# APRIL-ZJU/Ctrl-VIO

Measured on AMD Instinct MI355X. Metric: sliding-window solves/sec (10 KF, 200 lm, 2000 IMU), higher is better.
Workload: dtype f64; 1 GPU; config2: 10 KF / 200 landmarks / 2000 IMU sliding window (K = 24 knots, 814 reprojection blocks), <= 15 LM iterations (Ceres 1.14 trust region + projected line search); distinct_windows_per_gpu=64, streams_per_gpu=4, concurrent_solves_per_gpu=2

## Files before the change

ctrl-vio_amd/csrc/factors.hpp:

```cpp
#pragma once
#include "so3.hpp"

namespace ctv {

struct Knots4 {
  Q4 q[4];
  V3 p[4];
};

struct SegConst {
  V3 d[3];
  M3 JrI[3];
  CTV_DI M3 jri(int i) const { return JrI[i]; }
};
struct SegConstLazy {
  V3 d[3];
  const double *tab;
  CTV_DI M3 jri(int i) const {
    M3 J;
#pragma unroll
    for (int e = 0; e < 9; ++e) J.m[e] = tab[9 * i + e];
    return J;
  }
};
struct SegConstS {
  V3 d[3];
  M3 JrI[3];
  CTV_DI const M3 &jri(int i) const { return JrI[i]; }
};
CTV_DI void seg_const_lazy(const double *kd, const double *kjri, SegConstLazy &sc) {
#pragma unroll
  for (int i = 0; i < 3; ++i) sc.d[i] = mk(kd[3 * i], kd[3 * i + 1], kd[3 * i + 2]);
  sc.tab = kjri;
}
CTV_DI void seg_const(const Knots4 &k, SegConst &sc, bool want_jac) {
#pragma unroll
  for (int i = 0; i < 3; ++i) {
    sc.d[i] = so3_log(qmul(qconj(k.q[i]), k.q[i + 1]));
    if (want_jac) sc.JrI[i] = so3_Jr_inv(sc.d[i]);
  }
}

CTV_DI void knot_pair_const(const double *qa, const double *qb, double *d3, double *jri9) {
  const V3 dd = so3_log(qmul(qconj(qmk(qa[0], qa[1], qa[2], qa[3])), qmk(qb[0], qb[1], qb[2], qb[3])));
  d3[0] = dd.x; d3[1] = dd.y; d3[2] = dd.z;
  if (jri9) {
    const M3 J = so3_Jr_inv(mk(dd.x, dd.y, dd.z));
#pragma unroll
    for (int e = 0; e < 9; ++e) jri9[e] = J.m[e];
  }
}
CTV_DI void seg_const_load(const double *kd, const double *kjri, SegConst &sc, bool want_jac) {
#pragma unroll
  for (int i = 0; i < 3; ++i) {
    sc.d[i] = mk(kd[3 * i], kd[3 * i + 1], kd[3 * i + 2]);
    if (want_jac) {
#pragma unroll
      for (int e = 0; e < 9; ++e) sc.JrI[i].m[e] = kjri[9 * i + e];
    }
  }
}

struct ImuJac {
  M3 Jw[4], Ja[4];
  M3 Rinv_g;
  double lamA[4];
};

template <class SC> 
CTV_DI void imu_eval_core(const Knots4 &k, const SC &sc, double u, double idt, V3 gravity, const double bias[6],
                          const double gyro[3], const double acc[3], const double w[6], const M3 &RrefT, double r[6], bool want_jac, ImuJac &J) {
  double lamR[4], lamW[4];
  double (&lamA)[4] = J.lamA;
  basis<false, 2>(u, idt * idt, lamA);
  basis<true, 0>(u, 1.0, lamR);
  basis<true, 1>(u, idt, lamW);

  V3 accel = mk(0, 0, 0);
#pragma unroll
  for (int i = 0; i < 4; ++i) accel = accel + lamA[i] * k.p[i];

  Q4 Ainv[3], accq = qmk(0, 0, 0, 1);
  M3 Apost[4], JrK[3];
  Apost[3] = m3_id();
#pragma unroll
  for (int i = 2; i >= 0; --i) {
    const V3 nkd = (-lamR[i + 1]) * sc.d[i];
    Ainv[i] = so3_exp(nkd);
    accq = qmul_unit(accq, Ainv[i]);
    if (want_jac) { Apost[i] = q2R(accq); JrK[i] = so3_Jr(nkd); }
  }
  V3 om[4];
  om[0] = mk(0, 0, 0);
#pragma unroll
  for (int i = 0; i < 3; ++i) om[i + 1] = qrot(Ainv[i], om[i]) + lamW[i + 1] * sc.d[i];

  const Q4 Rinv_q = qmul_unit(accq, qconj(k.q[0]));
  const V3 ag = accel + gravity;
  const V3 a_pred = qrot(Rinv_q, ag);
  r[0] = w[0] * (om[3].x - (gyro[0] - bias[0]));
  r[1] = w[1] * (om[3].y - (gyro[1] - bias[1]));
  r[2] = w[2] * (om[3].z - (gyro[2] - bias[2]));
  r[3] = w[3] * (a_pred.x - (acc[0] - bias[3]));
  r[4] = w[4] * (a_pred.y - (acc[1] - bias[4]));
  r[5] = w[5] * (a_pred.z - (acc[2] - bias[5]));
  if (!want_jac) return;

  M3 (&Jw)[4] = J.Jw;
  M3 (&Ja)[4] = J.Ja;
#pragma unroll
  for (int i = 0; i < 4; ++i) { Jw[i] = m3_zero(); Ja[i] = m3_zero(); }
  {
    M3 dod = scale(Apost[1], lamW[1]);
#pragma unroll
    for (int i = 0; i < 3; ++i) {
      if (i > 0) dod = add(scale(mul(mul_hat(Apost[i], om[i]), JrK[i]), lamR[i + 1]), scale(Apost[i + 1], lamW[i + 1]));
      const M3 JrIi = sc.jri(i);
      Jw[i] = sub(Jw[i], mulT(dod, JrIi));
      Jw[i + 1] = add(Jw[i + 1], mul(dod, JrIi));
    }
  }
  const M3 Rinv = q2R(Rinv_q);
  J.Rinv_g = mul(Rinv, RrefT);
  {
    const M3 lhs = mul_hat(Rinv, ag);
    M3 Racc = q2R(k.q[0]);
    Ja[0] = add(Ja[0], mul(lhs, Racc));
#pragma unroll
    for (int i = 0; i < 3; ++i) {
      if (i > 0) Racc = mulT(Racc, q2R(Ainv[i - 1]));
      const M3 dad = scale(mul(mul(lhs, Racc), JrK[i]), lamR[i + 1]);
      const M3 JrIi = sc.jri(i);
      Ja[i] = sub(Ja[i], mulT(dad, JrIi));
      Ja[i + 1] = add(Ja[i + 1], mul(dad, JrIi));
    }
  }
}

CTV_DI void imu_row_gyro2(const M3 (&Jw)[4], const double w[6], const double r[6], int a, double out[16]) {
#pragma unroll
  for (int kk = 0; kk < 4; ++kk)
#pragma unroll
    for (int b = 0; b < 3; ++b) out[3 * kk + b] = w[a] * Jw[kk].m[3 * a + b];
  out[12] = out[13] = out[14] = 0.0;
  out[12 + a] = w[a];
  out[15] = r[a];
}

struct ImuMid3 {
  M3 Apost[3];
  M3 JrK[3];
  V3 om1, om2;
  V3 b[3];
  double lamR[4], lamW[4], lamA[4];
};
template <class SC> 
CTV_DI void imu_eval_values3(const double *gc, const SC &sc, double u, double idt, const double gyro[3], const double acc[3], const double w[6], double r[6], ImuMid3 &md) {
  basis<false, 2>(u, idt * idt, md.lamA);
  basis<true, 0>(u, 1.0, md.lamR);
  basis<true, 1>(u, idt, md.lamW);
  V3 ag = mk(gc[21], gc[22], gc[23]);
#pragma unroll
  for (int i = 1; i < 4; ++i) ag = ag + md.lamA[i] * mk(gc[3 * i], gc[3 * i + 1], gc[3 * i + 2]);
  Q4 Ainv[3], accq;
#pragma unroll
  for (int i = 2; i >= 0; --i) {
    const V3 nkd = (-md.lamR[i + 1]) * sc.d[i];
    Ainv[i] = so3_exp_small(nkd);
    accq = i == 2 ? Ainv[2] : qmul_unit(accq, Ainv[i]);
    md.Apost[i] = q2R(accq);
    md.JrK[i] = so3_Jr_small(nkd);
  }
  V3 om3;
  md.om1 = md.lamW[1] * sc.d[0];
  md.om2 = qrot(Ainv[1], md.om1) + md.lamW[2] * sc.d[1];
  om3 = qrot(Ainv[2], md.om2) + md.lamW[3] * sc.d[2];
  md.b[0] = mk(gc[12] * ag.x + gc[13] * ag.y + gc[14] * ag.z, gc[15] * ag.x + gc[16] * ag.y + gc[17] * ag.z,
                  gc[18] * ag.x + gc[19] * ag.y + gc[20] * ag.z);
  md.b[1] = qrot(Ainv[0], md.b[0]);
  md.b[2] = qrot(Ainv[1], md.b[1]);
  const V3 a_pred = qrot(Ainv[2], md.b[2]);
  r[0] = w[0] * (om3.x - (gyro[0] - gc[24]));
  r[1] = w[1] * (om3.y - (gyro[1] - gc[25]));
  r[2] = w[2] * (om3.z - (gyro[2] - gc[26]));
  r[3] = w[3] * (a_pred.x - (acc[0] - gc[27]));
  r[4] = w[4] * (a_pred.y - (acc[1] - gc[28]));
  r[5] = w[5] * (a_pred.z - (acc[2] - gc[29]));
}
template <class SC> CTV_DI void imu_apply_pair(const M3 &M, const SC &sc, int i, M3 &Ji, M3 &Ji1, bool first) {
  const M3 JrIi = sc.jri(i);
  const M3 A = mulT(M, JrIi), B = mul(M, JrIi);
#pragma unroll
  for (int e = 0; e < 9; ++e) { Ji.m[e] = first ? -A.m[e] : Ji.m[e] - A.m[e]; Ji1.m[e] = B.m[e]; }
}
template <class SC> CTV_DI void imu_jac_gyro3(const ImuMid3 &md, const SC &sc, M3 (&Jw)[4]) {
  imu_apply_pair(scale(md.Apost[1], md.lamW[1]), sc, 0, Jw[0], Jw[1], true);
  imu_apply_pair(add(scale(mul(mul_hat(md.Apost[1], md.om1), md.JrK[1]), md.lamR[2]), scale(md.Apost[2], md.lamW[2])), sc, 1, Jw[1], Jw[2], false);
  M3 dod = scale(mul(mul_hat(md.Apost[2], md.om2), md.JrK[2]), md.lamR[3]);
  dod.m[0] += md.lamW[3]; dod.m[4] += md.lamW[3]; dod.m[8] += md.lamW[3];
  imu_apply_pair(dod, sc, 2, Jw[2], Jw[3], false);
}
template <class SC> 
CTV_DI void imu_jac_accel3(const ImuMid3 &md, const SC &sc, const double *gc, M3 (&Ja)[4], M3 &Rinv_g) {
#pragma unroll
  for (int i = 0; i < 3; ++i)
#pragma unroll
    for (int j = 0; j < 3; ++j)
      Rinv_g.m[3 * i + j] = md.Apost[0].m[3 * i] * gc[12 + j] + md.Apost[0].m[3 * i + 1] * gc[15 + j] + md.Apost[0].m[3 * i + 2] * gc[18 + j];
  Ja[0] = mul_hat(md.Apost[0], md.b[0]);
#pragma unroll
  for (int i = 0; i < 3; ++i)
    imu_apply_pair(scale(mul(mul_hat(md.Apost[i], md.b[i]), md.JrK[i]), md.lamR[i + 1]), sc, i, Ja[i], Ja[i + 1], false);
}

CTV_DI void imu_row_accel3(const M3 (&Ja)[4], const double lamA[4], const M3 &Rinv_g, const double w[6], const double r[6], int a, double out[28]) {
#pragma unroll
  for (int kk = 0; kk < 4; ++kk)
#pragma unroll
    for (int b = 0; b < 3; ++b) {
      out[3 * kk + b] = w[3 + a] * Ja[kk].m[3 * a + b];
      out[16 + 3 * kk + b] = w[3 + a] * lamA[kk] * Rinv_g.m[3 * a + b];
    }
  out[12] = out[13] = out[14] = 0.0;
  out[12 + a] = w[3 + a];
  out[15] = r[3 + a];
}
template <class Sink> CTV_DI void imu_emit_cols(const ImuJac &J, const double w[6], Sink &sink) {
#pragma unroll
  for (int kk = 0; kk < 4; ++kk)
#pragma unroll
    for (int b = 0; b < 3; ++b) {
      double c6[6], p6[6];
#pragma unroll
      for (int a = 0; a < 3; ++a) {
        c6[a] = w[a] * J.Jw[kk].m[3 * a + b];
        c6[3 + a] = w[3 + a] * J.Ja[kk].m[3 * a + b];
        p6[a] = 0.0;
        p6[3 + a] = w[3 + a] * J.lamA[kk] * J.Rinv_g.m[3 * a + b];
      }
      sink.put_col(3 * kk + b, c6);
      sink.put_col(12 + 3 * kk + b, p6);
    }
#pragma unroll
  for (int a = 0; a < 3; ++a) {
    double g6[6] = {0.0, 0.0, 0.0, 0.0, 0.0, 0.0}, h6[6] = {0.0, 0.0, 0.0, 0.0, 0.0, 0.0};
    g6[a] = w[a];
    h6[3 + a] = w[3 + a];
    sink.put_col(24 + a, g6);
    sink.put_col(27 + a, h6);
  }
}
CTV_DI void imu_row_accel(const ImuJac &J, const double w[6], const double r[6], int a, double out[32]) {
#pragma unroll
  for (int kk = 0; kk < 4; ++kk)
#pragma unroll
    for (int b = 0; b < 3; ++b) {
      out[3 * kk + b] = w[3 + a] * J.Ja[kk].m[3 * a + b];
      out[12 + 3 * kk + b] = w[3 + a] * J.lamA[kk] * J.Rinv_g.m[3 * a + b];
    }
#pragma unroll
  for (int c = 24; c < 32; ++c) out[c] = 0.0;
  out[27 + a] = w[3 + a];
  out[30] = r[3 + a];
}
CTV_DI void imu_row_gyro(const ImuJac &J, const double w[6], const double r[6], int a, double out[16]) {
#pragma unroll
  for (int kk = 0; kk < 4; ++kk)
#pragma unroll
    for (int b = 0; b < 3; ++b) out[3 * kk + b] = w[a] * J.Jw[kk].m[3 * a + b];
  out[12] = out[13] = out[14] = 0.0;
  out[12 + a] = w[a];
  out[15] = r[a];
}

template <class Sink, class SC> 
CTV_DI void imu_eval(const Knots4 &k, const SC &sc, double u, double idt, V3 gravity, const double bias[6],
                     const double gyro[3], const double acc[3], const double w[6], const M3 &RrefT, double r[6], bool want_jac, Sink &sink) {
  ImuJac J;
  imu_eval_core<SC>(k, sc, u, idt, gravity, bias, gyro, acc, w, RrefT, r, want_jac, J);
  if (want_jac) imu_emit_cols(J, w, sink);
}

template <class SC, bool SMALL = false> CTV_DI Q4 eval_Rp(const Q4 q[4], const SC &sc, double u, M3 J[4], bool want_jac) {
  double c[4];
  basis<true, 0>(u, 1.0, c);
  Q4 accq = qmk(0, 0, 0, 1);
  M3 Apost[4], JrK[3];
  Apost[3] = m3_id();
#pragma unroll
  for (int i = 2; i >= 0; --i) {
    const V3 kd = c[i + 1] * sc.d[i];
    accq = qmul_unit(accq, so3_exp_sel<SMALL>(neg(kd)));
    if (want_jac) { JrK[i] = so3_Jr_sel<SMALL>(kd); Apost[i] = q2R(accq); }
  }
  const Q4 res = qmul_unit(q[0], qconj(accq));
  if (want_jac) {
    J[0] = Apost[0];
#pragma unroll
    for (int i = 0; i < 3; ++i) {
      const M3 Jh = scale(mul(Apost[i + 1], JrK[i]), c[i + 1]);
      J[i] = sub(J[i], mulT(Jh, sc.jri(i)));
      J[i + 1] = mul(Jh, sc.jri(i));
    }
  }
  return res;
}
template <class SC, bool SMALL = false> CTV_DI Q4 eval_RTp(const Q4 q[4], const SC &sc, double u, M3 J[4], bool want_jac) {
  double c[4];
  basis<true, 0>(u, 1.0, c);
  Q4 S[4];
  M3 JrK[3];
  S[0] = q[0];
#pragma unroll
  for (int i = 0; i < 3; ++i) {
    const V3 kd = c[i + 1] * sc.d[i];
    S[i + 1] = qmul_unit(S[i], so3_exp_sel<SMALL>(kd));
    if (want_jac) JrK[i] = so3_Jr_sel<SMALL>(neg(kd));
  }
  if (want_jac) {
    J[0] = q2R(S[0]);
#pragma unroll
    for (int i = 0; i < 3; ++i) {
      const M3 Jh = scale(mul(q2R(S[i]), JrK[i]), c[i + 1]);
      J[i] = sub(J[i], mulT(Jh, sc.jri(i)));
      J[i + 1] = mul(Jh, sc.jri(i));
    }
  }
  return qconj(S[3]);
}
template <class SC, bool SMALL = false> CTV_DI V3 eval_omega(const SC &sc, double u, double idt) {
  double c[4], dc[4];
  basis<true, 0>(u, 1.0, c);
  basis<true, 1>(u, idt, dc);
  V3 rv = dc[1] * sc.d[0];
#pragma unroll
  for (int i = 1; i < 3; ++i) rv = qrot(so3_exp_sel<SMALL>((-c[i + 1]) * sc.d[i]), rv) + dc[i + 1] * sc.d[i];
  return rv;
}
template <class SC> CTV_DI Q4 eval_R(const Q4 q[4], const SC &sc, double u) {
  double c[4];
  basis<true, 0>(u, 1.0, c);
  Q4 res = q[0];
#pragma unroll
  for (int i = 0; i < 3; ++i) res = qmul_unit(res, so3_exp(c[i + 1] * sc.d[i]));
  return res;
}

template <class SC> CTV_DI void pose_jac_T(const Q4 q[4], const SC &sc, double u, bool ext_on, Q4 q_SI, V3 p_SI, double *jt) {
  M3 J[4];
  const Q4 R = eval_Rp<SC>(q, sc, u, J, true);
  double c[4];
  basis<false, 0>(u, 1.0, c);
  M3 RSI = m3_id(), X = m3_zero();
  if (ext_on) { RSI = q2R(q_SI); X = scale(mul_hat(q2R(R), p_SI), -1.0); }
#pragma unroll
  for (int k = 0; k < 4; ++k) {
    const M3 B = mul(X, J[k]);
#pragma unroll
    for (int cc = 0; cc < 3; ++cc)
#pragma unroll
      for (int a = 0; a < 3; ++a) {
        jt[(6 * k + cc) * 6 + a] = ext_on ? RSI.m[a] * J[k].m[cc] + RSI.m[3 + a] * J[k].m[3 + cc] + RSI.m[6 + a] * J[k].m[6 + cc] : J[k].m[3 * a + cc];
        jt[(6 * k + cc) * 6 + 3 + a] = ext_on ? B.m[3 * a + cc] : 0.0;
        jt[(6 * k + 3 + cc) * 6 + a] = 0.0;
        jt[(6 * k + 3 + cc) * 6 + 3 + a] = a == cc ? c[k] : 0.0;
      }
  }
}

template <class SC> CTV_DI void nav_jac_T(const Q4 q[4], const SC &sc, double u, double idt, double *jt, double cv[4]) {
  pose_jac_T(q, sc, u, false, qmk(0.0, 0.0, 0.0, 1.0), mk(0.0, 0.0, 0.0), jt);
  basis<false, 1>(u, idt, cv);
}

CTV_DI void rel_pose_jac_T(Q4 q_a, V3 p_a, Q4 q_b, V3 p_b, double *jt_a, double *jt_b, Q4 &q_ab, V3 &p_ab) {
  q_ab = qmul(qconj(q_a), q_b);
  const M3 Ra = q2R(q_a), Rab = q2R(q_ab);
  const V3 d = p_b - p_a;
  p_ab = mk(Ra.m[0] * d.x + Ra.m[3] * d.y + Ra.m[6] * d.z, Ra.m[1] * d.x + Ra.m[4] * d.y + Ra.m[7] * d.z, Ra.m[2] * d.x + Ra.m[5] * d.y + Ra.m[8] * d.z);
  if (!jt_a) return;
  for (int r = 0; r < 24; ++r) {
    double *ja = jt_a + 6 * r, *jb = jt_b + 6 * r;
    const V3 th = mk(ja[0], ja[1], ja[2]), dp = mk(ja[3], ja[4], ja[5]), db = mk(jb[3], jb[4], jb[5]);
    const V3 x = cross(p_ab, th);
#pragma unroll
    for (int a = 0; a < 3; ++a) {
      ja[a] = -(Rab.m[a] * th.x + Rab.m[3 + a] * th.y + Rab.m[6 + a] * th.z);
      ja[3 + a] = (a == 0 ? x.x : a == 1 ? x.y : x.z) - (Ra.m[a] * dp.x + Ra.m[3 + a] * dp.y + Ra.m[6 + a] * dp.z);
      jb[3 + a] = Ra.m[a] * db.x + Ra.m[3 + a] * db.y + Ra.m[6 + a] * db.z;
    }
  }
}

template <class SC, bool SMALL = false, class F> CTV_DI void eval_Rp_jac_stream(const SC &sc, double u, F &&f) {
  double c[4];
  basis<true, 0>(u, 1.0, c);
  Q4 accq = qmk(0, 0, 0, 1);
  M3 Ap = m3_id(), pending = m3_zero();
#pragma unroll
  for (int i = 2; i >= 0; --i) {
    const V3 kd = c[i + 1] * sc.d[i];
    const M3 Jh = scale(mul(Ap, so3_Jr_sel<SMALL>(kd)), c[i + 1]);
    const M3 JrIi = sc.jri(i);
    const M3 Jn = mul(Jh, JrIi);
    f(i + 1, i == 2 ? Jn : add(Jn, pending));
    pending = scale(mulT(Jh, JrIi), -1.0);
    accq = qmul_unit(accq, so3_exp_sel<SMALL>(neg(kd)));
    Ap = q2R(accq);
  }
  f(0, add(Ap, pending));
}
template <class SC, bool SMALL = false, class F> CTV_DI void eval_RTp_jac_stream(const Q4 q[4], const SC &sc, double u, F &&f) {
  double c[4];
  basis<true, 0>(u, 1.0, c);
  Q4 S = q[0];
  M3 pending = q2R(S);
#pragma unroll
  for (int i = 0; i < 3; ++i) {
    const V3 kd = c[i + 1] * sc.d[i];
    const M3 Jh = scale(mul(q2R(S), so3_Jr_sel<SMALL>(neg(kd))), c[i + 1]);
    const M3 JrIi = sc.jri(i);
    f(i, sub(pending, mulT(Jh, JrIi)));
    pending = mul(Jh, JrIi);
    S = qmul_unit(S, so3_exp_sel<SMALL>(kd));
  }
  f(3, pending);
}

constexpr int AREC = 50;
constexpr int AR_PG = 0;
constexpr int AR_GR = 3;
constexpr int AR_CP0 = 39;
constexpr int AR_Y = 43;
constexpr int AR_H = 46;

template <bool SMALL, class SC>
CTV_DI void vis_anchor_eval(const Q4 &q0, const V3 p[4], const SC &sc, double u, double idt, const Q4 &q_CI,
                            const V3 &p_CI, double pix, double piy, double rowi, double d_inv, bool want_jac, double *rec) {
  const double inv_d = 1.0 / d_inv;
  const V3 c_i = qrot(q_CI, mk(pix * inv_d, piy * inv_d, inv_d));
  const V3 p_Ii = c_i + p_CI;
  Q4 qk[4];
  qk[0] = q0;
  const Q4 S_IitoG = eval_Rp<SC, SMALL>(qk, sc, u, (M3 *)nullptr, false);
  const M3 RIiG = q2R(S_IitoG);
  double cp0[4];
  basis<false, 0>(u, 1.0, cp0);
  V3 pI = mk(0, 0, 0);
#pragma unroll
  for (int i = 0; i < 4; ++i) pI = pI + cp0[i] * p[i];
  const V3 pG = mul(RIiG, p_Ii) + pI;
  rec[AR_PG] = pG.x; rec[AR_PG + 1] = pG.y; rec[AR_PG + 2] = pG.z;
  if (!want_jac) return;
  double dcp0[4];
  basis<false, 1>(u, idt, dcp0);
  V3 v_i = mk(0, 0, 0);
#pragma unroll
  for (int i = 0; i < 4; ++i) v_i = v_i + dcp0[i] * p[i];
#pragma unroll
  for (int i = 0; i < 4; ++i) rec[AR_CP0 + i] = cp0[i];
  const V3 y = (-inv_d) * mul(RIiG, c_i);
  rec[AR_Y] = y.x; rec[AR_Y + 1] = y.y; rec[AR_Y + 2] = y.z;
  const V3 Om_i = eval_omega<SC, SMALL>(sc, u, idt);
  const V3 h = rowi * (v_i + mul(RIiG, cross(Om_i, p_Ii)));
  rec[AR_H] = h.x; rec[AR_H + 1] = h.y; rec[AR_H + 2] = h.z;
  const M3 M0 = scale(mul_hat(RIiG, p_Ii), -1.0);
  eval_Rp_jac_stream<SC, SMALL>(sc, u, [&](int kk, const M3 &Jk) {
    const M3 G = mul(M0, Jk);
#pragma unroll
    for (int b = 0; b < 3; ++b)
#pragma unroll
      for (int mm = 0; mm < 3; ++mm) rec[AR_GR + 3 * (3 * kk + b) + mm] = G.m[3 * mm + b];
  });
}

constexpr int VB_JROT = 0;
constexpr int VB_RHO = 24;
constexpr int VB_LD = 26;
constexpr int VB_RES = 28;
constexpr int VB_AT = 30;
constexpr int VB_CP1 = 36;

template <bool SMALL, class SC, class Emit>
CTV_DI double vis_block_eval(const double *rec, const Q4 &q0, const V3 p[4], const SC &sc, double u, double idt,
                             const M3 &RCIT, const V3 &p_CI, double sw, double cauchy_a, double pjx, double pjy, double rowj,
                             double r[2], bool want_jac, Emit &emit) {
  double c[4], cp1[4];
  basis<true, 0>(u, 1.0, c);
  basis<false, 0>(u, 1.0, cp1);
  Q4 A[3], S[4];
  S[0] = q0;
#pragma unroll
  for (int i = 0; i < 3; ++i) {
    A[i] = so3_exp_sel<SMALL>(c[i + 1] * sc.d[i]);
    S[i + 1] = qmul_unit(S[i], A[i]);
  }
  const Q4 S_GtoIj = qconj(S[3]);
  V3 pIj = mk(0, 0, 0);
#pragma unroll
  for (int i = 0; i < 4; ++i) pIj = pIj + cp1[i] * p[i];
  const V3 dpg = mk(rec[AR_PG], rec[AR_PG + 1], rec[AR_PG + 2]) - pIj;
  const V3 bj = qrot(S_GtoIj, dpg);
  const V3 x_j = mul(RCIT, bj - p_CI);
  const double dji = 1.0 / x_j.z;
  const double r0 = sw * (x_j.x * dji - pjx), r1 = sw * (x_j.y * dji - pjy);
  const double s = r0 * r0 + r1 * r1;
  double cost, sq = 1.0, rs = 1.0, alpha_sq = 0.0;
  if (cauchy_a > 0.0) {
    const double b = cauchy_a * cauchy_a, cc = 1.0 / b;
    const double inv = 1.0 / (1.0 + s * cc);
    cost = 0.5 * b * log1p(s * cc);
    const double rho1 = inv, rho2 = -cc * inv * inv;
    sq = sqrt(rho1);
    if (s == 0.0 || rho2 <= 0.0) { rs = sq; alpha_sq = 0.0; }
    else { const double D = 1.0 + 2.0 * s * rho2 / rho1; const double al = 1.0 - sqrt(D); rs = sq / (1.0 - al); alpha_sq = al / s; }
  } else {
    cost = 0.5 * s;
  }
  r[0] = rs * r0;
  r[1] = rs * r1;
  if (!want_jac) return cost;
  double Bt[6], At[6];
  {
    const double fx = -dji * dji * x_j.x, fy = -dji * dji * x_j.y;
#pragma unroll
    for (int k = 0; k < 3; ++k) {
      const double j0 = sw * (dji * RCIT.m[k] + fx * RCIT.m[6 + k]), j1 = sw * (dji * RCIT.m[3 + k] + fy * RCIT.m[6 + k]);
      const double rj = r0 * j0 + r1 * j1;
      Bt[k] = sq * (j0 - alpha_sq * r0 * rj);
      Bt[3 + k] = sq * (j1 - alpha_sq * r1 * rj);
    }
  }
  const M3 RGIj = q2R(S_GtoIj);
#pragma unroll
  for (int a = 0; a < 2; ++a)
#pragma unroll
    for (int k = 0; k < 3; ++k) At[3 * a + k] = Bt[3 * a] * RGIj.m[k] + Bt[3 * a + 1] * RGIj.m[3 + k] + Bt[3 * a + 2] * RGIj.m[6 + k];
  emit.put(VB_RHO, At[0] * rec[AR_Y] + At[1] * rec[AR_Y + 1] + At[2] * rec[AR_Y + 2]);
  emit.put(VB_RHO + 1, At[3] * rec[AR_Y] + At[4] * rec[AR_Y + 1] + At[5] * rec[AR_Y + 2]);
#pragma unroll
  for (int mm = 0; mm < 3; ++mm) { emit.put(VB_AT + 2 * mm, At[mm]); emit.put(VB_AT + 2 * mm + 1, At[3 + mm]); }
#pragma unroll
  for (int i = 0; i < 4; ++i) emit.put(VB_CP1 + i, cp1[i]);
  {
    double dc[4], dcp1[4];
    basis<true, 1>(u, idt, dc);
    basis<false, 1>(u, idt, dcp1);
    V3 v_j = mk(0, 0, 0);
#pragma unroll
    for (int i = 0; i < 4; ++i) v_j = v_j + dcp1[i] * p[i];
    V3 Om_j = dc[1] * sc.d[0];
#pragma unroll
    for (int i = 1; i < 3; ++i) Om_j = qrot(qconj(A[i]), Om_j) + dc[i + 1] * sc.d[i];
    const V3 hv = mk(rec[AR_H], rec[AR_H + 1], rec[AR_H + 2]) - rowj * v_j;
    const V3 Jx = qrot(S_GtoIj, hv) - rowj * cross(Om_j, bj);
    emit.put(VB_LD, Bt[0] * Jx.x + Bt[1] * Jx.y + Bt[2] * Jx.z);
    emit.put(VB_LD + 1, Bt[3] * Jx.x + Bt[4] * Jx.y + Bt[5] * Jx.z);
  }
  {
    const V3 E0 = cross(mk(At[0], At[1], At[2]), dpg), E1 = cross(mk(At[3], At[4], At[5]), dpg);
    const double E[6] = {E0.x, E0.y, E0.z, E1.x, E1.y, E1.z};
    auto mul23 = [](const double X[6], const M3 &M, double Y[6]) {
#pragma unroll
      for (int a = 0; a < 2; ++a)
#pragma unroll
        for (int k = 0; k < 3; ++k) Y[3 * a + k] = X[3 * a] * M.m[k] + X[3 * a + 1] * M.m[3 + k] + X[3 * a + 2] * M.m[6 + k];
    };
    auto mul23T = [](const double X[6], const M3 &M, double Y[6]) {
#pragma unroll
      for (int a = 0; a < 2; ++a)
#pragma unroll
        for (int k = 0; k < 3; ++k) Y[3 * a + k] = X[3 * a] * M.m[3 * k] + X[3 * a + 1] * M.m[3 * k + 1] + X[3 * a + 2] * M.m[3 * k + 2];
    };
    double Ep[6];
    mul23(E, q2R(S[0]), Ep);
#pragma unroll
    for (int i = 0; i < 3; ++i) {
      double ER[6], EH[6], t6[6];
      if (i == 0) {
#pragma unroll
        for (int e = 0; e < 6; ++e) ER[e] = Ep[e];
      } else {
        mul23(E, q2R(S[i]), ER);
      }
      mul23(ER, so3_Jr_sel<SMALL>((-c[i + 1]) * sc.d[i]), EH);
#pragma unroll
      for (int e = 0; e < 6; ++e) EH[e] *= c[i + 1];
      const M3 JrIi = sc.jri(i);
      mul23T(EH, JrIi, t6);
#pragma unroll
      for (int b = 0; b < 3; ++b) {
        emit.put(VB_JROT + 2 * (3 * i + b), Ep[b] - t6[b]);
        emit.put(VB_JROT + 2 * (3 * i + b) + 1, Ep[3 + b] - t6[3 + b]);
      }
      mul23(EH, JrIi, Ep);
    }
#pragma unroll
    for (int b = 0; b < 3; ++b) { emit.put(VB_JROT + 2 * (9 + b), Ep[b]); emit.put(VB_JROT + 2 * (9 + b) + 1, Ep[3 + b]); }
  }
  return cost;
}

}
```

ctrl-vio_amd/csrc/kernels_visual.hpp:

```cpp
#pragma once

namespace ctv {

__device__ __forceinline__ void vis_times(const WinMeta &m, long long t_rel, int row, double ld, int &s, double &u) {
  const long long ld_ns = (long long)(ld * 1e9);
  const long long tau = t_rel + (long long)row * ld_ns;
  s = (int)(tau / m.dt_ns);
  u = (double)(tau % m.dt_ns) / (double)m.dt_ns;
}

constexpr int AREC_LD = AREC + 1;
__device__ __forceinline__ void vis_anchor_body(const Dev &d, int mode, double *srec , int block) {
  const int a = block * 64 + threadIdx.x;
  bool run = false;
  if (a < d.Atot) run = lin_run(d.lm[d.a_win[a]], mode);
  const unsigned long long run_mask = __ballot(run);
  if (run_mask == 0) return;
  if (run) {
  const int w = d.a_win[a];
  const Lm &lm = d.lm[w];
  const WinMeta &m = d.wins[w];
  const bool jac = !lin_cost_only(lm, mode, d.prm);
  const bool at_cand = mode == LIN_SPEC;
  const double *quat = at_cand ? d.cquat : d.quat, *pos = at_cand ? d.cpos : d.pos, *rho = at_cand ? d.crho : d.rho, *ldp = at_cand ? d.cld : d.ld;
  int si;
  double ui;
  const int rowi = d.a_row[a];
  vis_times(m, d.a_t[a], rowi, ldp[w], si, ui);
  si = max(0, min(si, m.K - 4));
  SegConstLazy sc;
  seg_const_lazy(d.lkd + 3 * (m.knot0 + si), d.kjri + 9 * (m.knot0 + si), sc);
  double dmax = 0.0;
#pragma unroll
  for (int i = 0; i < 3; ++i) dmax = fmax(dmax, dot(sc.d[i], sc.d[i]));
  const bool small = __ballot(dmax >= 0.25) == 0ull;
  const double *qi = quat + 4 * (m.knot0 + si), *pi = pos + 3 * (m.knot0 + si);
  const Q4 q0 = qmk(qi[0], qi[1], qi[2], qi[3]);
  V3 p[4];
#pragma unroll
  for (int i = 0; i < 4; ++i) p[i] = mk(pi[3 * i], pi[3 * i + 1], pi[3 * i + 2]);
  const Q4 q_CI = qmk(m.q_CI[0], m.q_CI[1], m.q_CI[2], m.q_CI[3]);
  const V3 p_CI = mk(m.p_CI[0], m.p_CI[1], m.p_CI[2]);
  double *rec = srec + AREC_LD * threadIdx.x;
  if (!jac)
    for (int e = 0; e < AREC; ++e) rec[e] = 0.0;
  const double pix = d.a_obs[a], piy = d.a_obs[(size_t)d.Atot + a], d_inv = rho[m.lm0 + d.a_lm[a]];
  if (small) vis_anchor_eval<true>(q0, p, sc, ui, m.inv_dt, q_CI, p_CI, pix, piy, (double)rowi, d_inv, jac, rec);
  else vis_anchor_eval<false>(q0, p, sc, ui, m.inv_dt, q_CI, p_CI, pix, piy, (double)rowi, d_inv, jac, rec);
  d.a_s[a] = si;
  }
  lds_wave_sync();
  {
    const int lane = threadIdx.x;
    double *dst = d.arec + (size_t)(block * 64) * AREC;
    constexpr int HP = AREC / 2;
#pragma unroll 5
    for (int k = 0; k < HP; ++k) {
      const int i = k * 64 + lane, bl = i / HP, r = 2 * (i - bl * HP);
      VecN<double, 2> pr;
      pr.v[0] = srec[AREC_LD * bl + r];
      pr.v[1] = srec[AREC_LD * bl + r + 1];
      if ((run_mask >> bl) & 1ull) *reinterpret_cast<VecN<double, 2> *>(dst + (size_t)bl * AREC + r) = pr;
    }
  }
}
__global__ __launch_bounds__(64) void k_vis_anchor(Dev d, int mode) {
  __shared__ __attribute__((aligned(16))) double srec[64 * AREC_LD];
  vis_anchor_body(d, mode, srec, blockIdx.x);
}

__device__ __forceinline__ int vt_at(int l, int e) { return VT_ROWS * l + (e ^ ((l >> 2) & 7)); }
struct VisRecSink {
  double *wcs;
  int l;
  __device__ __forceinline__ void put(int e, double v) { wcs[vt_at(l, e)] = v; }
};
struct VisNullSink {
  __device__ __forceinline__ void put(int, double) {}
};

constexpr int VIS_LDS_BYTES = 64 * VT_ROWS * 8;
constexpr int VIS_ROW_BYTES = VIS_LDS_BYTES - 64 * 16;
__device__ __forceinline__ void vis_eval_body(const Dev &d, int mode, unsigned char *smt, int vblock) {
  const int v = vblock * 64 + threadIdx.x;
  const long long t_entry = d.dbg ? clock64() : 0ll;
  constexpr int LDS_BYTES = VIS_ROW_BYTES;
  long long *rowoff = reinterpret_cast<long long *>(smt + VIS_ROW_BYTES);
  int *rlm = reinterpret_cast<int *>(rowoff + 64), *rspan = rlm + 64;
  double *wcs = reinterpret_cast<double *>(smt);
  const bool at_cand = mode == LIN_SPEC;
  const double *quat = at_cand ? d.cquat : d.quat, *pos = at_cand ? d.cpos : d.pos, *ldp = at_cand ? d.cld : d.ld;
  double c = 0.0;
  int ksj = 0, my_lm = -1, my_anc = -1;
  bool on = false, costed = false;
  const int wu = d.vb_win[vblock];
  const Lm &lmw = d.lm[wu];
  const WinMeta &m = d.wins[wu];
  if (!lin_run(lmw, mode)) return;
  const bool jac = !lin_cost_only(lmw, mode, d.prm);
  const int tgw = lin_target(lmw, mode);
  if (v < d.Vtot && d.v_win[v] >= 0) {
    {
      int sj;
      double uj;
      const int rowj = d.v_rowj[v];
      vis_times(m, d.v_tj[v], rowj, ldp[wu], sj, uj);
      sj = max(0, min(sj, m.K - 4));
      SegConstLazy scj;
      seg_const_lazy(d.lkd + 3 * (m.knot0 + sj), d.kjri + 9 * (m.knot0 + sj), scj);
      double dmax = 0.0;
#pragma unroll
      for (int i = 0; i < 3; ++i) dmax = fmax(dmax, dot(scj.d[i], scj.d[i]));
      const bool small = __ballot(dmax >= 0.25) == 0ull;
      const double *qj = quat + 4 * (m.knot0 + sj), *pj = pos + 3 * (m.knot0 + sj);
      const Q4 q0 = qmk(qj[0], qj[1], qj[2], qj[3]);
      V3 p[4];
#pragma unroll
      for (int i = 0; i < 4; ++i) p[i] = mk(pj[3 * i], pj[3 * i + 1], pj[3 * i + 2]);
      const int anc = d.v_anc[v];
      const double *rec = reinterpret_cast<const double *>(__builtin_assume_aligned(d.arec + (size_t)anc * AREC, 16));
      M3 RCIT;
      {
        const M3 R = q2R(qmk(m.q_CI[0], m.q_CI[1], m.q_CI[2], m.q_CI[3]));
#pragma unroll
        for (int a = 0; a < 3; ++a)
#pragma unroll
          for (int b = 0; b < 3; ++b) RCIT.m[3 * a + b] = R.m[3 * b + a];
      }
      const V3 p_CI = mk(m.p_CI[0], m.p_CI[1], m.p_CI[2]);
      const double pjx = d.v_obs[v], pjy = d.v_obs[(size_t)d.Vtot + v], ca = d.v_cauchy[v];
      double r[2];
      if (jac) {
        VisRecSink sink{wcs, (int)threadIdx.x};
        on = true;
        my_lm = d.v_lm[v];
        my_anc = anc;
        if (small) c = vis_block_eval<true>(rec, q0, p, scj, uj, m.inv_dt, RCIT, p_CI, m.img_w, ca, pjx, pjy, (double)rowj, r, true, sink);
        else c = vis_block_eval<false>(rec, q0, p, scj, uj, m.inv_dt, RCIT, p_CI, m.img_w, ca, pjx, pjy, (double)rowj, r, true, sink);
        sink.put(VB_RES, r[0]); sink.put(VB_RES + 1, r[1]);
        d.vsj[v] = sj;
        ksj = sj;
      } else {
        VisNullSink nsink;
        costed = true;
        c = vis_block_eval<false>(rec, q0, p, scj, uj, m.inv_dt, RCIT, p_CI, m.img_w, ca, pjx, pjy, (double)rowj, r, false, nsink);
      }
    }
  }
  {
    const int lane = threadIdx.x;
    const unsigned long long on_mask = __ballot(on);
    if (on_mask != 0 || __any(costed)) {
      double cs = c;
#pragma unroll
      for (int off = 32; off > 0; off >>= 1) cs += __shfl_xor(cs, off);
      if (lane == 0) d.vis_cost[vblock] = cs;
    }
    if (on_mask == 0) return;
    const int P = m.P, ldw = m.ldw, lm0 = m.lm0, u0 = m.u0;
    const long long W0 = m.W0;
    double *Wset = d.WS[tgw];
    double *Hllset = d.HllS[tgw], *gset = d.gS[tgw];
    long long *dbg = (d.dbg && vblock == 1000) ? d.dbg + 32 : nullptr;
    if (dbg && lane == 0) { dbg[-1] = t_entry; dbg[0] = clock64() + (long long)(c * 0); }
    lds_wave_sync();
    double wj[24], s6[6];
    {
      auto Jl = [&](int e) { return wcs[vt_at(lane, e)]; };
      const double jr0 = Jl(VB_RHO), jr1 = Jl(VB_RHO + 1);
#pragma unroll
      for (int cc = 0; cc < 12; ++cc) wj[cc] = jr0 * Jl(VB_JROT + 2 * cc) + jr1 * Jl(VB_JROT + 2 * cc + 1);
#pragma unroll
      for (int b = 0; b < 3; ++b) s6[b] = jr0 * Jl(VB_AT + 2 * b) + jr1 * Jl(VB_AT + 2 * b + 1);
#pragma unroll
      for (int k = 0; k < 4; ++k) {
        const double cp1 = Jl(VB_CP1 + k);
#pragma unroll
        for (int b = 0; b < 3; ++b) wj[12 + 3 * k + b] = -(cp1 * s6[b]);
      }
      s6[3] = jr0 * Jl(VB_LD) + jr1 * Jl(VB_LD + 1);
      s6[4] = jr0 * jr0 + jr1 * jr1;
      s6[5] = jr0 * Jl(VB_RES) + jr1 * Jl(VB_RES + 1);
    }
    double hg[40];
    int ksi, my_row, my_klo, my_khi;
    {
      const double *rec = reinterpret_cast<const double *>(__builtin_assume_aligned(d.arec + (size_t)max(my_anc, 0) * AREC, 16));
#pragma unroll
      for (int e = 0; e < 40; ++e) hg[e] = rec[AR_GR + e];
      ksi = d.a_s[max(my_anc, 0)];
      my_row = d.lm_pos[lm0 + max(my_lm, 0)];
      my_klo = d.lm_klo[lm0 + my_row]; my_khi = d.lm_khi[lm0 + my_row];
    }
    const int prev_lm = __shfl_up(my_lm, 1), prev_anc = __shfl_up(my_anc, 1);
    const bool head = on && (lane == 0 || prev_lm != my_lm), head_a = on && (lane == 0 || prev_anc != my_anc);
    const unsigned long long heads = __ballot(head), heads_a = __ballot(head_a);
    const int ord = __popcll(heads & ((2ull << lane) - 1ull)) - 1;
    const int nlm = __popcll(heads);
    const int ha = 63 - __clzll((long long)(heads_a & ((2ull << lane) - 1ull)));
    int maxlen = on ? lane - ha + 1 : 0;
#pragma unroll
    for (int off = 32; off > 0; off >>= 1) maxlen = max(maxlen, __shfl_xor(maxlen, off));
    maxlen = __builtin_amdgcn_readfirstlane(maxlen);
    for (int off = 1; off < maxlen; off <<= 1) {
      const int oh = __shfl_down(on ? ha : -1, off);
      const bool take = on && (lane + off < 64) && oh == ha;
#pragma unroll
      for (int cc = 0; cc < 6; ++cc) { const double o = __shfl_down(s6[cc], off); s6[cc] += take ? o : 0.0; }
    }
    if (dbg && lane == 0) dbg[1] = clock64() + (long long)(s6[0] * 0);
    {
      double *dst = d.Jt + (size_t)(vblock * 64) * VT_ROWS;
      constexpr int HP = VT_ROWS / 2;
#pragma unroll 4
      for (int k = 0; k < HP; ++k) {
        const int i = k * 64 + lane, bl = i / HP, r = 2 * (i - bl * HP);
        const int sw = (bl >> 2) & 7;
        const VecN<double, 2> pp = *reinterpret_cast<const VecN<double, 2> *>(wcs + VT_ROWS * bl + (r ^ (sw & 6)));
        VecN<double, 2> pr;
        pr.v[0] = (sw & 1) ? pp.v[1] : pp.v[0];
        pr.v[1] = (sw & 1) ? pp.v[0] : pp.v[1];
        if ((on_mask >> bl) & 1ull) *reinterpret_cast<VecN<double, 2> *>(dst + (size_t)bl * VT_ROWS + r) = pr;
      }
    }
    if (dbg && lane == 0) dbg[2] = clock64();
    double wi[24];
#pragma unroll
    for (int k = 0; k < 4; ++k)
#pragma unroll
      for (int b = 0; b < 3; ++b) {
        const int cc = 3 * k + b;
        wi[cc] = s6[0] * hg[3 * cc] + s6[1] * hg[3 * cc + 1] + s6[2] * hg[3 * cc + 2];
        wi[12 + cc] = hg[36 + k] * s6[b];
      }
    double *rows = reinterpret_cast<double *>(smt);
    const int SPW = d.max_span6;
    const int RS = SPW + 3;
    const int NR = max(1, min(nlm, ((int)(LDS_BYTES / 8) - 1) / RS));
    int ri = ksi - my_klo, rj = ksj - my_klo;
    if (on && (rj < 0 || ksj + 3 > my_khi || (head_a && (ri < 0 || ksi + 3 > my_khi)))) atomicAdd(d.span_viol, 1);
    ri = max(0, min(ri, SPW / 6 - 4)); rj = max(0, min(rj, SPW / 6 - 4));
    lds_wave_sync();
    if (head) { rowoff[ord] = W0 + (long long)my_row * ldw; rlm[ord] = my_lm; rspan[ord] = (my_klo << 16) | max(my_khi - my_klo + 1, 0); }
    for (int c0 = 0; c0 < nlm; c0 += NR) {
      const int nr = min(NR, nlm - c0);
      for (int i = 2 * lane; i < nr * RS; i += 128) *reinterpret_cast<VecN<double, 2> *>(rows + i) = VecN<double, 2>{{0.0, 0.0}};
      lds_wave_sync();
      if (on && ord >= c0 && ord < c0 + nr) {
        double *row = rows + (size_t)(ord - c0) * RS;
        if (head_a) {
#pragma unroll
          for (int k = 0; k < 4; ++k)
#pragma unroll
            for (int b = 0; b < 3; ++b) {
              atomicAdd(&row[6 * (ri + k) + b], wi[3 * k + b]);
              atomicAdd(&row[6 * (ri + k) + 3 + b], wi[12 + 3 * k + b]);
            }
          atomicAdd(&row[SPW], s6[3]);
          atomicAdd(&row[SPW + 1], s6[4]);
          atomicAdd(&row[SPW + 2], s6[5]);
        }
#pragma unroll
        for (int k = 0; k < 4; ++k)
#pragma unroll
          for (int b = 0; b < 3; ++b) {
            atomicAdd(&row[6 * (rj + k) + b], wj[3 * k + b]);
            atomicAdd(&row[6 * (rj + k) + 3 + b], wj[12 + 3 * k + b]);
          }
      }
      lds_wave_sync();
      if (dbg && lane == 0) dbg[3 + 2 * (c0 / NR)] = clock64();
      {
        for (int rb = 0; rb < nr; rb += 4) {
          const int q = rb + (lane >> 4);
          if (q < nr) {
            const int sp = rspan[c0 + q], k0 = sp >> 16, npair = 3 * (sp & 0xffff);
            double *Wr = Wset + rowoff[c0 + q] + 6 * k0;
            const double *row = rows + (size_t)q * RS;
            for (int cp = lane & 15; cp < npair; cp += 16) {
              VecN<double, 2> rv;
              rv.v[0] = row[2 * cp]; rv.v[1] = row[2 * cp + 1];
              *reinterpret_cast<VecN<double, 2> *>(Wr + 2 * cp) = rv;
            }
          }
        }
        if (lane < nr) {
          const double *row = rows + (size_t)lane * RS;
          const int l = rlm[c0 + lane];
          Wset[rowoff[c0 + lane] + P - 1] = row[SPW];
          Hllset[lm0 + l] = row[SPW + 1];
          gset[u0 + P + l] = row[SPW + 2];
        }
      }
      lds_wave_sync();
      if (dbg && lane == 0) { dbg[4 + 2 * (c0 / NR)] = clock64(); dbg[10] = nlm * 1000000ll; dbg[11] = NR * 1000; }
    }
  }
}

__global__ __launch_bounds__(64) __attribute__((amdgpu_waves_per_eu(2))) void k_vis_eval(Dev d, int mode) {
  __shared__ __attribute__((aligned(16))) unsigned char smt[VIS_LDS_BYTES];
  vis_eval_body(d, mode, smt, blockIdx.x);
}

__global__ __launch_bounds__(64) __attribute__((amdgpu_waves_per_eu(1, 1))) void k_linearize_f64(Dev d, int mode, int general_only, int zero_mode) {
  static_assert(VIS_LDS_BYTES >= (72 * 33 + 64) * 8, "the IMU rows use the head of the visual body's LDS buffer");
  __shared__ __attribute__((aligned(32))) unsigned char smt[VIS_LDS_BYTES];
  if ((int)blockIdx.x < d.Gtot) {
    if (!general_only) imu_linearize_f64_fast(d, mode, reinterpret_cast<double *>(smt), blockIdx.x, d.Gtot, zero_mode);
  } else vis_eval_body(d, mode, smt, blockIdx.x - d.Gtot);
}

}
```

Before: 50200 solves/s.

## Stage anchor records through swizzled LDS in two rounds to shrink shared memory

```diff
diff --git a/ctrl-vio_amd/csrc/factors.hpp b/ctrl-vio_amd/csrc/factors.hpp
--- a/ctrl-vio_amd/csrc/factors.hpp
+++ b/ctrl-vio_amd/csrc/factors.hpp
@@ -434,9 +434,9 @@
 constexpr int AR_Y = 43;
 constexpr int AR_H = 46;
 
-template <bool SMALL, class SC>
-CTV_DI void vis_anchor_eval(const Q4 &q0, const V3 p[4], const SC &sc, double u, double idt, const Q4 &q_CI,
-                            const V3 &p_CI, double pix, double piy, double rowi, double d_inv, bool want_jac, double *rec) {
+template <bool SMALL, class SC, class Rec>
+CTV_DI void vis_anchor_emit(const Q4 &q0, const V3 p[4], const SC &sc, double u, double idt, const Q4 &q_CI,
+                            const V3 &p_CI, double pix, double piy, double rowi, double d_inv, bool want_jac, Rec &rec) {
   const double inv_d = 1.0 / d_inv;
   const V3 c_i = qrot(q_CI, mk(pix * inv_d, piy * inv_d, inv_d));
   const V3 p_Ii = c_i + p_CI;
@@ -450,7 +450,7 @@
 #pragma unroll
   for (int i = 0; i < 4; ++i) pI = pI + cp0[i] * p[i];
   const V3 pG = mul(RIiG, p_Ii) + pI;
-  rec[AR_PG] = pG.x; rec[AR_PG + 1] = pG.y; rec[AR_PG + 2] = pG.z;
+  rec.put(AR_PG, pG.x); rec.put(AR_PG + 1, pG.y); rec.put(AR_PG + 2, pG.z);
   if (!want_jac) return;
   double dcp0[4];
   basis<false, 1>(u, idt, dcp0);
@@ -458,20 +458,31 @@
 #pragma unroll
   for (int i = 0; i < 4; ++i) v_i = v_i + dcp0[i] * p[i];
 #pragma unroll
-  for (int i = 0; i < 4; ++i) rec[AR_CP0 + i] = cp0[i];
+  for (int i = 0; i < 4; ++i) rec.put(AR_CP0 + i, cp0[i]);
   const V3 y = (-inv_d) * mul(RIiG, c_i);
-  rec[AR_Y] = y.x; rec[AR_Y + 1] = y.y; rec[AR_Y + 2] = y.z;
+  rec.put(AR_Y, y.x); rec.put(AR_Y + 1, y.y); rec.put(AR_Y + 2, y.z);
   const V3 Om_i = eval_omega<SC, SMALL>(sc, u, idt);
   const V3 h = rowi * (v_i + mul(RIiG, cross(Om_i, p_Ii)));
-  rec[AR_H] = h.x; rec[AR_H + 1] = h.y; rec[AR_H + 2] = h.z;
+  rec.put(AR_H, h.x); rec.put(AR_H + 1, h.y); rec.put(AR_H + 2, h.z);
   const M3 M0 = scale(mul_hat(RIiG, p_Ii), -1.0);
   eval_Rp_jac_stream<SC, SMALL>(sc, u, [&](int kk, const M3 &Jk) {
     const M3 G = mul(M0, Jk);
 #pragma unroll
     for (int b = 0; b < 3; ++b)
 #pragma unroll
-      for (int mm = 0; mm < 3; ++mm) rec[AR_GR + 3 * (3 * kk + b) + mm] = G.m[3 * mm + b];
+      for (int mm = 0; mm < 3; ++mm) rec.put(AR_GR + 3 * (3 * kk + b) + mm, G.m[3 * mm + b]);
   });
+}
+
+struct ArecArray {
+  double *rec;
+  CTV_DI void put(int e, double v) { rec[e] = v; }
+};
+template <bool SMALL, class SC>
+CTV_DI void vis_anchor_eval(const Q4 &q0, const V3 p[4], const SC &sc, double u, double idt, const Q4 &q_CI,
+                            const V3 &p_CI, double pix, double piy, double rowi, double d_inv, bool want_jac, double *rec) {
+  ArecArray out{rec};
+  vis_anchor_emit<SMALL>(q0, p, sc, u, idt, q_CI, p_CI, pix, piy, rowi, d_inv, want_jac, out);
 }
 
 constexpr int VB_JROT = 0;
diff --git a/ctrl-vio_amd/csrc/kernels_visual.hpp b/ctrl-vio_amd/csrc/kernels_visual.hpp
--- a/ctrl-vio_amd/csrc/kernels_visual.hpp
+++ b/ctrl-vio_amd/csrc/kernels_visual.hpp
@@ -9,13 +9,29 @@
   u = (double)(tau % m.dt_ns) / (double)m.dt_ns;
 }
 
+__device__ __forceinline__ int vt_at(int l, int e) { return VT_ROWS * l + (e ^ ((l >> 2) & 7)); }
+
 constexpr int AREC_LD = AREC + 1;
+constexpr int AR_SIDE0 = 2, AR_NSIDE = AREC - VT_ROWS;
+static_assert(AR_NSIDE == 10 && AR_SIDE0 % 2 == 0 && AR_SIDE0 + AR_NSIDE == AR_GR + 9, "the second round: p_G.z and GR of knot 0, five aligned pairs");
+struct AnchorRecSink {
+  double *stage;
+  int l;
+  double side[AR_NSIDE];
+  __device__ __forceinline__ void put(int e, double v) {
+    if (e >= AR_SIDE0 && e < AR_SIDE0 + AR_NSIDE) side[e - AR_SIDE0] = v;
+    else stage[vt_at(l, e < AR_SIDE0 ? e : e - AR_NSIDE)] = v;
+  }
+};
 __device__ __forceinline__ void vis_anchor_body(const Dev &d, int mode, double *srec , int block) {
   const int a = block * 64 + threadIdx.x;
   bool run = false;
   if (a < d.Atot) run = lin_run(d.lm[d.a_win[a]], mode);
   const unsigned long long run_mask = __ballot(run);
   if (run_mask == 0) return;
+  AnchorRecSink out;
+  out.stage = srec;
+  out.l = threadIdx.x;
   if (run) {
   const int w = d.a_win[a];
   const Lm &lm = d.lm[w];
@@ -41,35 +57,54 @@
   for (int i = 0; i < 4; ++i) p[i] = mk(pi[3 * i], pi[3 * i + 1], pi[3 * i + 2]);
   const Q4 q_CI = qmk(m.q_CI[0], m.q_CI[1], m.q_CI[2], m.q_CI[3]);
   const V3 p_CI = mk(m.p_CI[0], m.p_CI[1], m.p_CI[2]);
-  double *rec = srec + AREC_LD * threadIdx.x;
   if (!jac)
-    for (int e = 0; e < AREC; ++e) rec[e] = 0.0;
+    for (int e = 0; e < VT_ROWS; ++e) srec[vt_at(out.l, e)] = 0.0;
   const double pix = d.a_obs[a], piy = d.a_obs[(size_t)d.Atot + a], d_inv = rho[m.lm0 + d.a_lm[a]];
-  if (small) vis_anchor_eval<true>(q0, p, sc, ui, m.inv_dt, q_CI, p_CI, pix, piy, (double)rowi, d_inv, jac, rec);
-  else vis_anchor_eval<false>(q0, p, sc, ui, m.inv_dt, q_CI, p_CI, pix, piy, (double)rowi, d_inv, jac, rec);
+  if (small) vis_anchor_emit<true>(q0, p, sc, ui, m.inv_dt, q_CI, p_CI, pix, piy, (double)rowi, d_inv, jac, out);
+  else vis_anchor_emit<false>(q0, p, sc, ui, m.inv_dt, q_CI, p_CI, pix, piy, (double)rowi, d_inv, jac, out);
   d.a_s[a] = si;
+  if (!jac) {
+#pragma unroll
+    for (int e = AR_GR; e < AR_SIDE0 + AR_NSIDE; ++e) out.put(e, 0.0);
+  }
   }
   lds_wave_sync();
+  const int lane = threadIdx.x;
+  double *dst = d.arec + (size_t)(block * 64) * AREC;
   {
-    const int lane = threadIdx.x;
-    double *dst = d.arec + (size_t)(block * 64) * AREC;
-    constexpr int HP = AREC / 2;
+    constexpr int HP = VT_ROWS / 2;
 #pragma unroll 5
     for (int k = 0; k < HP; ++k) {
       const int i = k * 64 + lane, bl = i / HP, r = 2 * (i - bl * HP);
+      const int sw = (bl >> 2) & 7;
+      const VecN<double, 2> pp = *reinterpret_cast<const VecN<double, 2> *>(srec + VT_ROWS * bl + (r ^ (sw & 6)));
       VecN<double, 2> pr;
-      pr.v[0] = srec[AREC_LD * bl + r];
-      pr.v[1] = srec[AREC_LD * bl + r + 1];
-      if ((run_mask >> bl) & 1ull) *reinterpret_cast<VecN<double, 2> *>(dst + (size_t)bl * AREC + r) = pr;
-    }
-  }
-}
-__global__ __launch_bounds__(64) void k_vis_anchor(Dev d, int mode) {
-  __shared__ __attribute__((aligned(16))) double srec[64 * AREC_LD];
+      pr.v[0] = (sw & 1) ? pp.v[1] : pp.v[0];
+      pr.v[1] = (sw & 1) ? pp.v[0] : pp.v[1];
+      if ((run_mask >> bl) & 1ull) *reinterpret_cast<VecN<double, 2> *>(dst + (size_t)bl * AREC + (r < AR_SIDE0 ? r : r + AR_NSIDE)) = pr;
+    }
+  }
+  lds_wave_sync();
+  {
+    constexpr int SP = AR_NSIDE / 2, SLD = AR_NSIDE + 1;
+#pragma unroll
+    for (int e = 0; e < AR_NSIDE; ++e) srec[SLD * lane + e] = out.side[e];
+    lds_wave_sync();
+#pragma unroll
+    for (int k = 0; k < SP; ++k) {
+      const int i = k * 64 + lane, bl = i / SP, q = i - bl * SP;
+      VecN<double, 2> pr;
+      pr.v[0] = srec[SLD * bl + 2 * q];
+      pr.v[1] = srec[SLD * bl + 2 * q + 1];
+      if ((run_mask >> bl) & 1ull) *reinterpret_cast<VecN<double, 2> *>(dst + (size_t)bl * AREC + AR_SIDE0 + 2 * q) = pr;
+    }
+  }
+}
+__global__ __launch_bounds__(64) __attribute__((amdgpu_waves_per_eu(2))) void k_vis_anchor(Dev d, int mode) {
+  __shared__ __attribute__((aligned(16))) double srec[64 * VT_ROWS];
   vis_anchor_body(d, mode, srec, blockIdx.x);
 }
 
-__device__ __forceinline__ int vt_at(int l, int e) { return VT_ROWS * l + (e ^ ((l >> 2) & 7)); }
 struct VisRecSink {
   double *wcs;
   int l;
```

New measurement: 50170 solves/s. Within noise of the previous version (-0.1%).
